# glacierbliss/iceberg_tracking_code

Hardware: AMD Instinct MI355X
Metric: frame_pairs_per_sec (higher is better)
Workload: dtype u8/int32/f32

## Files before the change

### iceberg_tracking_code_amd/csrc/k_corners.hip

```cpp
#include <algorithm>
#include <cstdlib>

#include "icelk_internal.h"

namespace icelk {

namespace {

__device__ __forceinline__ int reflect101(int p, int n)
{
    if (n == 1) return 0;
    while (p < 0 || p >= n) p = p < 0 ? -p : 2 * n - 2 - p;
    return p;
}

__device__ __forceinline__ unsigned ordered_key(float v)
{
    const unsigned b = __float_as_uint(v);
    return (b & 0x80000000u) ? ~b : (b | 0x80000000u);
}
__device__ __forceinline__ float key_to_float(unsigned k)
{
    const unsigned b = (k & 0x80000000u) ? (k & 0x7fffffffu) : ~k;
    return __uint_as_float(b);
}

__device__ __forceinline__ unsigned pack_xy(int x, int y) { return ((unsigned)y << 16) | (unsigned)x; }

__device__ __forceinline__ float threshold_of(const unsigned* max_key, double quality)
{
    const unsigned mk = *max_key;
    const double max_val = mk ? (double)key_to_float(mk) : 0.0;
    return (float)(max_val * quality);
}

__device__ __forceinline__ float row_smooth(float a, float b, float c, float k0, float k1, int variant)
{
    if (variant & 2) return fmaf(k1, c, fmaf(k0, b, __fmul_rn(k1, a)));
    return __fadd_rn(__fadd_rn(__fmul_rn(k1, a), __fmul_rn(k0, b)), __fmul_rn(k1, c));
}

__device__ __forceinline__ void sobel_cov(float a0, float b0, float c0, float a1, float c1, float a2, float b2,
                                          float c2, float k0, float k1, float& xx, float& xy, float& yy, int variant = 0)
{
    const float dx = (variant & 1) ? fmaf(__fadd_rn(__fsub_rn(c0, a0), __fsub_rn(c2, a2)), k1, __fmul_rn(__fsub_rn(c1, a1), k0))
                                   : __fadd_rn(__fmul_rn(__fadd_rn(__fsub_rn(c0, a0), __fsub_rn(c2, a2)), k1),
                                               __fmul_rn(__fsub_rn(c1, a1), k0));
    const float t0 = row_smooth(a0, b0, c0, k0, k1, variant);
    const float t2 = row_smooth(a2, b2, c2, k0, k1, variant);
    const float dy = __fsub_rn(t2, t0);
    xx = __fmul_rn(dx, dx);
    xy = __fmul_rn(dx, dy);
    yy = __fmul_rn(dy, dy);
}

typedef float f2 __attribute__((ext_vector_type(2)));
__device__ __forceinline__ void sobel_cov2(f2 a0, f2 b0, f2 c0, f2 a1, f2 c1, f2 a2, f2 b2, f2 c2, float k0, float k1,
                                           f2& xx, f2& xy, f2& yy)
{
    const f2 dx = ((c0 - a0) + (c2 - a2)) * k1 + (c1 - a1) * k0;
    const f2 t0 = (a0 * k1 + b0 * k0) + c0 * k1;
    const f2 t2 = (a2 * k1 + b2 * k0) + c2 * k1;
    const f2 dy = t2 - t0;
    xx = dx * dx;
    xy = dx * dy;
    yy = dy * dy;
}

template <int N, int BS>
__device__ __forceinline__ void window_sums(const double (&v)[N + BS - 1], double (&out)[N])
{
    if constexpr (BS <= 3) {
#pragma unroll
        for (int i = 0; i < N; i++) {
            double s = 0;
#pragma unroll
            for (int k = 0; k < BS; k++) s += v[i + k];
            out[i] = s;
        }
    } else {
        double s = v[0];
#pragma unroll
        for (int k = 1; k < BS; k++) s += v[k];
        out[0] = s;
#pragma unroll
        for (int i = 1; i < N; i++) {
            s = (s - v[i - 1]) + v[i + BS - 1];
            out[i] = s;
        }
    }
}

__device__ __forceinline__ float min_eig_of(double s0, double s1, double s2, int variant = 0)
{
    const float a = __fmul_rn((float)s0, 0.5f), b = (float)s1, c = __fmul_rn((float)s2, 0.5f);
    const float d = __fsub_rn(a, c);
    const float r = (variant & 4) ? fmaf(b, b, __fmul_rn(d, d)) : __fadd_rn(__fmul_rn(d, d), __fmul_rn(b, b));
    return __fsub_rn(__fadd_rn(a, c), sqrtf(r));
}

__device__ __forceinline__ void publish_max(unsigned* max_key, unsigned best, int tid)
{
#pragma unroll
    for (int o = 32; o >= 1; o >>= 1) {
        const unsigned other = __shfl_xor(best, o);
        best = other > best ? other : best;
    }
    if ((tid & 63) == 0 && best > __atomic_load_n(max_key, __ATOMIC_RELAXED)) atomicMax(max_key, best);
}

struct CandSrc {
    const unsigned long long* keys;
    const int* blk_count;
    int nblk;
    int region;
};

constexpr int gcd_c(int a, int b) { return b == 0 ? a : gcd_c(b, a % b); }

template <int BS>
struct StripCfg {
    static constexpr int NT = 256;
    static constexpr int AN = BS / 2;
    static constexpr int EW = NT - (BS - 1);
    static constexpr int TW = EW - 2;
    static constexpr int R = 4;
    static constexpr int UNROLL = BS * R / gcd_c(BS, R);
    static constexpr int EH = (64 / UNROLL) * UNROLL;
    static constexpr int SH = EH - 2;
    static constexpr int NROWS = EH + BS - 1;
    static constexpr int RX = 4;
    static constexpr int NG = (EW + RX - 1) / RX;
    static constexpr int VP = NT + 2;
    static constexpr int SUB = 16, NSUB = (SH + SUB - 1) / SUB;
    static constexpr int V_BYTES = R * 3 * VP * 8;
    static constexpr int E_BYTES = 8 * NT * 4;
    static constexpr int LDS_BYTES = V_BYTES + E_BYTES;
    static_assert(EH % R == 0 && NG <= 64 && RX * NG <= NT + RX - 1, "one wave per row of a batch");
    static_assert(RX * (NG - 1) + RX + BS - 2 < VP, "row tasks stay inside a row of column sums");
    static_assert((VP * 8) % 16 == 0, "16-byte reads of the column sums");
};

struct SobelRoll {
    float d1, d2, t1, t2;
};

__device__ __forceinline__ float smooth3(float a, float b, float c, float k0, float k1)
{
    return __fadd_rn(__fadd_rn(__fmul_rn(k1, a), __fmul_rn(k0, b)), __fmul_rn(k1, c));
}

template <int BS, bool FRESH>
__device__ __forceinline__ void strip_body(const uint8_t* __restrict__ img, int w, int h, int pitch, float k0, float k1,
                                           const uint8_t* __restrict__ mask, int mask_pitch, unsigned* __restrict__ max_key,
                                           unsigned long long* __restrict__ raw, int* __restrict__ blk_count,
                                           float* __restrict__ eig_out, uint8_t* smem, int* s_cnt)
{
    using C = StripCfg<BS>;
    double* Vb = reinterpret_cast<double*>(smem);
    float* Er = reinterpret_cast<float*>(smem + C::V_BYTES);
    const int tid = threadIdx.x;
    const int x0 = blockIdx.x * C::TW, y0 = blockIdx.y * C::SH;
    const int xs = x0 - 1 - C::AN, ys = y0 - 1 - C::AN;
    const int rx = reflect101(xs + tid, w);
    const int xm = reflect101(rx - 1, w), xp = reflect101(rx + 1, w);
    const int bid = blockIdx.y * gridDim.x + blockIdx.x;
    if (tid < C::NSUB) s_cnt[tid] = 0;

    float ring[3][BS];
#pragma unroll
    for (int k = 0; k < BS; k++) ring[0][k] = ring[1][k] = ring[2][k] = 0.f;
    double V[3] = {0.0, 0.0, 0.0};
    SobelRoll S{};
    unsigned pa = 0, pb = 0, pc = 0;
    if (!FRESH) {
        const uint8_t* r2 = img + (size_t)(ys - 1) * pitch;
        const uint8_t* r1 = r2 + pitch;
        const uint8_t* r0 = r1 + pitch;
        const float a2 = (float)r2[xm], b2 = (float)r2[rx], c2 = (float)r2[xp];
        const float a1 = (float)r1[xm], b1 = (float)r1[rx], c1 = (float)r1[xp];
        S.d2 = __fsub_rn(c2, a2); S.t2 = smooth3(a2, b2, c2, k0, k1);
        S.d1 = __fsub_rn(c1, a1); S.t1 = smooth3(a1, b1, c1, k0, k1);
        pa = r0[xm]; pb = r0[rx]; pc = r0[xp];
    }
    auto cov_row = [&](int r, float& xx, float& xy, float& yy) {
        float dtop, dmid, dbot, ttop, tbot;
        if (FRESH) {
            const int ry = reflect101(ys + r, h);
            const uint8_t* q0 = img + (size_t)reflect101(ry - 1, h) * pitch;
            const uint8_t* q1 = img + (size_t)ry * pitch;
            const uint8_t* q2 = img + (size_t)reflect101(ry + 1, h) * pitch;
            const float a0 = (float)q0[xm], b0 = (float)q0[rx], c0 = (float)q0[xp];
            const float a1 = (float)q1[xm], c1 = (float)q1[xp];
            const float a2 = (float)q2[xm], b2 = (float)q2[rx], c2 = (float)q2[xp];
            dtop = __fsub_rn(c0, a0); dmid = __fsub_rn(c1, a1); dbot = __fsub_rn(c2, a2);
            ttop = smooth3(a0, b0, c0, k0, k1); tbot = smooth3(a2, b2, c2, k0, k1);
        } else {
            const float a = (float)pa, b = (float)pb, c = (float)pc;
            int nr = ys + r + 2;
            nr = nr < h ? nr : h - 1;
            const uint8_t* q = img + (size_t)nr * pitch;
            pa = q[xm]; pb = q[rx]; pc = q[xp];
            dtop = S.d2; dmid = S.d1; dbot = __fsub_rn(c, a);
            ttop = S.t2; tbot = smooth3(a, b, c, k0, k1);
            S.d2 = S.d1; S.d1 = dbot; S.t2 = S.t1; S.t1 = tbot;
        }
        const float dx = __fadd_rn(__fmul_rn(__fadd_rn(dtop, dbot), k1), __fmul_rn(dmid, k0));
        const float dy = __fsub_rn(tbot, ttop);
        xx = __fmul_rn(dx, dx); xy = __fmul_rn(dx, dy); yy = __fmul_rn(dy, dy);
    };

#pragma unroll
    for (int r = 0; r < BS - 1; r++) {
        float p[3];
        cov_row(r, p[0], p[1], p[2]);
#pragma unroll
        for (int q = 0; q < 3; q++) { V[q] += (double)p[q]; ring[q][r] = p[q]; }
    }

    unsigned best = 0;
    const int wr = tid >> 6, g = tid & 63;
    for (int base = 0; base < C::EH; base += C::UNROLL) {
#pragma unroll
        for (int j = 0; j < C::UNROLL; j++) {
            const int i = base + j;
            const int K = (BS - 1 + j) % BS;
            float p[3];
            cov_row(BS - 1 + i, p[0], p[1], p[2]);
#pragma unroll
            for (int q = 0; q < 3; q++) {
                V[q] = (V[q] + (double)p[q]) - (double)ring[q][K];
                ring[q][K] = p[q];
                Vb[((j % C::R) * 3 + q) * C::VP + tid] = V[q];
            }
            __builtin_amdgcn_sched_barrier(0);
            if (j % C::R != C::R - 1) continue;
            const int eb = i / C::R;
            __syncthreads();
            if (g < C::NG && wr < C::R) {
                double Sm[3][C::RX];
#pragma unroll
                for (int q = 0; q < 3; q++) {
                    double v[C::RX + BS - 1];
                    const double* src = Vb + (wr * 3 + q) * C::VP + C::RX * g;
#pragma unroll
                    for (int k = 0; k < C::RX + BS - 1; k++) v[k] = src[k];
                    window_sums<C::RX, BS>(v, Sm[q]);
                    __builtin_amdgcn_sched_barrier(0);
                }
                const int er = eb * C::R + wr;
                float e[C::RX];
#pragma unroll
                for (int k = 0; k < C::RX; k++) e[k] = min_eig_of(Sm[0][k], Sm[1][k], Sm[2][k]);
                *reinterpret_cast<float4*>(Er + (er & 7) * C::NT + C::RX * g) = make_float4(e[0], e[1], e[2], e[3]);
                const int y = y0 - 1 + er;
                if (er >= 1 && er <= C::SH && y < h) {
#pragma unroll
                    for (int k = 0; k < C::RX; k++) {
                        const int ce = C::RX * g + k, x = x0 - 1 + ce;
                        if (ce >= 1 && ce <= C::TW && x < w) {
                            if (eig_out) eig_out[(size_t)y * w + x] = e[k];
                            if (!mask || mask[(size_t)y * mask_pitch + x]) {
                                const unsigned key = ordered_key(e[k]);
                                best = key > best ? key : best;
                            }
                        }
                    }
                }
            }
            __syncthreads();
            {
                const int x = x0 - 1 + tid;
                if (tid >= 1 && tid <= C::TW && x >= 1 && x < w - 1) {
                    float m3[6], mid[6], side[6];
#pragma unroll
                    for (int k = 0; k < 6; k++) {
                        const float* row = Er + ((eb * C::R - 2 + k) & 7) * C::NT + tid;
                        const float l = row[-1], c = row[0], r = row[1];
                        mid[k] = c;
                        side[k] = fmaxf(l, r);
                        m3[k] = fmaxf(side[k], c);
                    }
#pragma unroll
                    for (int q = 0; q < 4; q++) {
                        const int c = eb * C::R - 1 + q, y = y0 - 1 + c;
                        if (c < 1 || c > C::SH || y < 1 || y >= h - 1) continue;
                        const float v = mid[q + 1];
                        if (!(v > 0.f)) continue;
                        const float m = fmaxf(fmaxf(m3[q], m3[q + 2]), side[q + 1]);
                        if (v < m) continue;
                        if (mask && !mask[(size_t)y * mask_pitch + x]) continue;
                        const int sub = (c - 1) / C::SUB;
                        const int pos = atomicAdd(&s_cnt[sub], 1);
                        raw[((size_t)bid * C::NSUB + sub) * (C::TW * C::SUB) + pos] =
                            ((unsigned long long)ordered_key(v) << 32) | pack_xy(x, y);
                    }
                }
            }
        }
    }
    publish_max(max_key, best, tid);
    __syncthreads();
    if (tid < C::NSUB) blk_count[bid * C::NSUB + tid] = s_cnt[tid];
}

template <int BS>
__global__ __launch_bounds__(256) __attribute__((amdgpu_waves_per_eu(3, 4))) void k_eig_strip(const uint8_t* __restrict__ img, int w, int h, int pitch, float k0,
                                                    float k1, const uint8_t* __restrict__ mask, int mask_pitch,
                                                    unsigned* __restrict__ max_key,
                                                    unsigned long long* __restrict__ raw, int* __restrict__ blk_count,
                                                    float* __restrict__ eig_out)
{
    using C = StripCfg<BS>;
    extern __shared__ __attribute__((aligned(16))) uint8_t smem[];
    __shared__ int s_cnt[C::NSUB];
    const int ys = (int)blockIdx.y * C::SH - 1 - C::AN;
    if (ys - 1 >= 0 && ys + C::NROWS <= h - 1)
        strip_body<BS, false>(img, w, h, pitch, k0, k1, mask, mask_pitch, max_key, raw, blk_count, eig_out, smem, s_cnt);
    else
        strip_body<BS, true>(img, w, h, pitch, k0, k1, mask, mask_pitch, max_key, raw, blk_count, eig_out, smem, s_cnt);
}

__device__ __forceinline__ void block_append(bool keep, unsigned long long key, unsigned long long* out,
                                             int* out_count, int* s_cnt, int* s_base)
{
    if (threadIdx.x == 0) *s_cnt = 0;
    __syncthreads();
    const int pos = keep ? atomicAdd(s_cnt, 1) : 0;
    __syncthreads();
    if (threadIdx.x == 0 && *s_cnt) *s_base = atomicAdd(out_count, *s_cnt);
    __syncthreads();
    if (keep) out[*s_base + pos] = key;
    __syncthreads();
}

__global__ __launch_bounds__(256) void k_flatten(CandSrc src, const unsigned* __restrict__ max_key, double quality,
                                                 unsigned long long* __restrict__ cand, int* __restrict__ cand_count)
{
    __shared__ int s_cnt, s_base;
    const float thr = threshold_of(max_key, quality);
    for (int b = blockIdx.x; b < src.nblk; b += gridDim.x) {
        const int cnt = src.blk_count[b];
        for (int i0 = 0; i0 < cnt; i0 += 256) {
            const int i = i0 + threadIdx.x;
            unsigned long long key = 0;
            bool keep = false;
            if (i < cnt) {
                key = src.keys[(size_t)b * src.region + i];
                keep = key_to_float((unsigned)(key >> 32)) > thr;
            }
            block_append(keep, key, cand, cand_count, &s_cnt, &s_base);
        }
    }
}

constexpr int EIG_TW = 64;
constexpr int EIG_TH = 16;

__global__ __launch_bounds__(256) void k_min_eig(const uint8_t* __restrict__ img, int w, int h, int pitch, int bs,
                                                 float k0, float k1, float* __restrict__ eig,
                                                 const uint8_t* __restrict__ mask, int mask_pitch,
                                                 unsigned* __restrict__ max_key, int variant)
{
    extern __shared__ __attribute__((aligned(16))) uint8_t smem[];
    const int anchor = bs / 2;
    const int ew = EIG_TW + bs - 1, eh = EIG_TH + bs - 1;
    double* hs = reinterpret_cast<double*>(smem);
    float* cov = reinterpret_cast<float*>(smem + sizeof(double) * 3 * eh * EIG_TW);
    const int x0 = blockIdx.x * EIG_TW, y0 = blockIdx.y * EIG_TH;
    const int tid = threadIdx.x;
    for (int i = tid; i < ew * eh; i += 256) {
        const int ey = i / ew, ex = i - ey * ew;
        const int rx = reflect101(x0 - anchor + ex, w), ry = reflect101(y0 - anchor + ey, h);
        const int xm = reflect101(rx - 1, w), xp = reflect101(rx + 1, w);
        const int ym = reflect101(ry - 1, h), yp = reflect101(ry + 1, h);
        const uint8_t* r0 = img + (size_t)ym * pitch;
        const uint8_t* r1 = img + (size_t)ry * pitch;
        const uint8_t* r2 = img + (size_t)yp * pitch;
        float xx, xy, yy;
        sobel_cov((float)r0[xm], (float)r0[rx], (float)r0[xp], (float)r1[xm], (float)r1[xp], (float)r2[xm],
                  (float)r2[rx], (float)r2[xp], k0, k1, xx, xy, yy, variant);
        cov[i] = xx;
        cov[ew * eh + i] = xy;
        cov[2 * ew * eh + i] = yy;
    }
    __syncthreads();
    for (int i = tid; i < eh * EIG_TW; i += 256) {
        const int ey = i / EIG_TW, ox = i - ey * EIG_TW;
        const float* c = cov + ey * ew + ox;
        double s0 = 0, s1 = 0, s2 = 0;
        for (int k = 0; k < bs; k++) {
            s0 += (double)c[k];
            s1 += (double)c[ew * eh + k];
            s2 += (double)c[2 * ew * eh + k];
        }
        hs[i] = s0;
        hs[eh * EIG_TW + i] = s1;
        hs[2 * eh * EIG_TW + i] = s2;
    }
    __syncthreads();
    unsigned best = 0;
    for (int i = tid; i < EIG_TH * EIG_TW; i += 256) {
        const int oy = i / EIG_TW, ox = i - oy * EIG_TW;
        const int x = x0 + ox, y = y0 + oy;
        if (x >= w || y >= h) continue;
        const double* r = hs + oy * EIG_TW + ox;
        double s0 = 0, s1 = 0, s2 = 0;
        for (int k = 0; k < bs; k++) {
            s0 += r[k * EIG_TW];
            s1 += r[eh * EIG_TW + k * EIG_TW];
            s2 += r[2 * eh * EIG_TW + k * EIG_TW];
        }
        const float v = min_eig_of(s0, s1, s2, variant);
        eig[(size_t)y * w + x] = v;
        if (!mask || mask[(size_t)y * mask_pitch + x]) {
            const unsigned k = ordered_key(v);
            best = k > best ? k : best;
        }
    }
    publish_max(max_key, best, tid);
}

constexpr int NMS_ROWS = 8;
__global__ __launch_bounds__(256) void k_nms_collect(const float* __restrict__ eig, int w, int h,
                                                     const uint8_t* __restrict__ mask, int mask_pitch,
                                                     const unsigned* __restrict__ max_key, double quality,
                                                     unsigned long long* __restrict__ raw, int* __restrict__ blk_count)
{
    __shared__ int list_n;
    const int tid = threadIdx.x;
    if (tid == 0) list_n = 0;
    __syncthreads();
    const int bid = blockIdx.y * gridDim.x + blockIdx.x;
    unsigned long long* region = raw + (size_t)bid * (256 * NMS_ROWS);
    const float thr = threshold_of(max_key, quality);
    const int x = blockIdx.x * 256 + tid + 1;
    for (int r = 0; r < NMS_ROWS; r++) {
        const int y = blockIdx.y * NMS_ROWS + r + 1;
        if (x >= w - 1 || y >= h - 1) continue;
        const float v = eig[(size_t)y * w + x];
        if (!(v > thr) || v == 0.f) continue;
        if (mask && !mask[(size_t)y * mask_pitch + x]) continue;
        float m = 0.f;
#pragma unroll
        for (int dy = -1; dy <= 1; dy++)
#pragma unroll
            for (int dx = -1; dx <= 1; dx++) {
                float q = eig[(size_t)(y + dy) * w + (x + dx)];
                q = q > thr ? q : 0.f;
                m = q > m ? q : m;
            }
        if (v != m) continue;
        region[atomicAdd(&list_n, 1)] = ((unsigned long long)ordered_key(v) << 32) | pack_xy(x, y);
    }
    __syncthreads();
    if (tid == 0) blk_count[bid] = list_n;
}

constexpr int CT = 64;
constexpr int SCAN_CHUNK = 2048;
constexpr int CHUNK_TOT_STRIDE = 32;

__device__ __forceinline__ void chunk_add(int* __restrict__ chunk_tot, bool active, int chunk)
{
    unsigned long long pending = __ballot(active);
    while (pending) {
        const int leader = __ffsll((long long)pending) - 1;
        const int c = __shfl(chunk, leader);
        const unsigned long long same = __ballot(active && chunk == c) & pending;
        if ((int)threadIdx.x == leader) atomicAdd(&chunk_tot[c * CHUNK_TOT_STRIDE], __popcll(same));
        pending &= ~same;
    }
}

__global__ __launch_bounds__(CT) void k_cell_count(CandSrc src, const unsigned* __restrict__ max_key, double quality,
                                                   const unsigned* __restrict__ prune_key, int w, int cell, int gw,
                                                   int* __restrict__ cell_count, int* __restrict__ chunk_tot)
{
    const float thr = threshold_of(max_key, quality);
    const unsigned pk = *prune_key;
    for (int b = blockIdx.x; b < src.nblk; b += gridDim.x) {
        const int cnt = src.blk_count[b];
        for (int i0 = 0; i0 < cnt; i0 += CT) {
            const int i = i0 + threadIdx.x;
            bool keep = false;
            int c = 0;
            if (i < cnt) {
                const unsigned long long key = src.keys[(size_t)b * src.region + i];
                keep = (unsigned)(key >> 32) >= pk && key_to_float((unsigned)(key >> 32)) > thr;
                const unsigned idx = (unsigned)key;
                const int y = (int)(idx >> 16), x = (int)(idx & 0xffffu);
                c = (y / cell) * gw + (x / cell);
            }
            if (keep) atomicAdd(&cell_count[c], 1);
            chunk_add(chunk_tot, keep, c / SCAN_CHUNK);
        }
    }
}

constexpr int KEY_SHIFT = 18;
constexpr int KEY_BINS = 2048;
__device__ __forceinline__ int key_bin(unsigned key, unsigned max_key)
{
    const int b = (int)(max_key >> KEY_SHIFT) - (int)(key >> KEY_SHIFT);
    return b < 0 ? 0 : (b >= KEY_BINS ? KEY_BINS - 1 : b);
}

__global__ __launch_bounds__(CT) void k_key_hist(CandSrc src, const unsigned* __restrict__ max_key, double quality,
                                                 unsigned* __restrict__ hist)
{
    __shared__ unsigned lh[KEY_BINS];
    for (int i = threadIdx.x; i < KEY_BINS; i += CT) lh[i] = 0;
    __syncthreads();
    const float thr = threshold_of(max_key, quality);
    const unsigned mk = *max_key;
    for (int b = blockIdx.x; b < src.nblk; b += gridDim.x) {
        const int cnt = src.blk_count[b];
        for (int i = threadIdx.x; i < cnt; i += CT) {
            const unsigned k = (unsigned)(src.keys[(size_t)b * src.region + i] >> 32);
            if (key_to_float(k) > thr) atomicAdd(&lh[key_bin(k, mk)], 1u);
        }
    }
    __syncthreads();
    for (int i = threadIdx.x; i < KEY_BINS; i += CT) {
        const unsigned v = lh[i];
        if (v) atomicAdd(&hist[i], v);
    }
}

__global__ __launch_bounds__(CT) void k_key_select(const unsigned* __restrict__ hist, unsigned want,
                                                   const unsigned* __restrict__ max_key,
                                                   unsigned* __restrict__ prune_key)
{
    constexpr int PER = KEY_BINS / CT;
    const int lane = threadIdx.x;
    unsigned s = 0;
    for (int i = 0; i < PER; i++) s += hist[lane * PER + i];
    unsigned incl = s;
#pragma unroll
    for (int o = 1; o < CT; o <<= 1) {
        const unsigned v = __shfl_up(incl, o);
        if (lane >= o) incl += v;
    }
    const unsigned total = __shfl(incl, CT - 1);
    if (lane == 0 && total < want) *prune_key = 0u;
    const unsigned above = incl - s;
    if (above < want && incl >= want) {
        unsigned run = above;
        for (int i = 0; i < PER; i++) {
            run += hist[lane * PER + i];
            if (run >= want) {
                const int bin = lane * PER + i;
                const int top = (int)(*max_key >> KEY_SHIFT);
                *prune_key = (bin >= KEY_BINS - 1 || top - bin <= 0) ? 0u : (unsigned)(top - bin) << KEY_SHIFT;
                break;
            }
        }
    }
}

__global__ __launch_bounds__(CT) void k_scan(const int* __restrict__ count, const int* __restrict__ chunk_tot,
                                             int* __restrict__ start, int n)
{
    const int lane = threadIdx.x;
    const int lo = blockIdx.x * SCAN_CHUNK;
    int run = 0;
    for (int c = lane; c < (int)blockIdx.x; c += CT) run += chunk_tot[c * CHUNK_TOT_STRIDE];
#pragma unroll
    for (int o = 32; o >= 1; o >>= 1) run += __shfl_xor(run, o);
    for (int r = 0; r < SCAN_CHUNK / (4 * CT); r++) {
        const int i0 = lo + r * 4 * CT + 4 * lane;
        int c[4], s = 0;
#pragma unroll
        for (int k = 0; k < 4; k++) {
            c[k] = i0 + k < n ? count[i0 + k] : 0;
            s += c[k];
        }
        int inc = s;
#pragma unroll
        for (int o = 1; o < CT; o <<= 1) {
            const int v = __shfl_up(inc, o);
            if (lane >= o) inc += v;
        }
        int at = run + inc - s;
#pragma unroll
        for (int k = 0; k < 4; k++) {
            if (i0 + k < n) start[i0 + k] = at;
            at += c[k];
            if (i0 + k == n - 1) start[n] = at;
        }
        run += __shfl(inc, CT - 1);
    }
    if (n == 0 && blockIdx.x == 0 && lane == 0) start[0] = 0;
}

__global__ __launch_bounds__(CT) void k_cell_fill(CandSrc src, const unsigned* __restrict__ max_key, double quality,
                                                   const unsigned* __restrict__ prune_key, int w, int cell, int gw,
                                                   const int* __restrict__ cell_start, int* __restrict__ cell_fill,
                                                   unsigned long long* __restrict__ cell_cand,
                                                   uint8_t* __restrict__ state)
{
    const float thr = threshold_of(max_key, quality);
    const unsigned pk = *prune_key;
    for (int b = blockIdx.x; b < src.nblk; b += gridDim.x) {
        const int cnt = src.blk_count[b];
        for (int i = threadIdx.x; i < cnt; i += CT) {
            const unsigned long long key = src.keys[(size_t)b * src.region + i];
            if ((unsigned)(key >> 32) < pk || !(key_to_float((unsigned)(key >> 32)) > thr)) continue;
            const unsigned idx = (unsigned)key;
            const int y = (int)(idx >> 16), x = (int)(idx & 0xffffu);
            const int c = (y / cell) * gw + (x / cell);
            const int pos = cell_start[c] + atomicAdd(&cell_fill[c], 1);
            cell_cand[pos] = key;
            state[pos] = 0;
        }
    }
}

constexpr int SUP_K = 24;
constexpr int SUP_SPINS = 48;
__global__ __launch_bounds__(CT) void k_suppress(const unsigned long long* __restrict__ cell_cand,
                                                  const int* __restrict__ n_ptr, int cell, int gw, int gh,
                                                  const int* __restrict__ cell_start, uint8_t* state, double md2,
                                                  int* __restrict__ launch_counters, int r)
{
    __shared__ int blockers[SUP_K * CT];
    if (r > 0 && launch_counters[r - 1] == 0) return;
    const int n = *n_ptr;
    int* mine = blockers + threadIdx.x;
    for (int i = blockIdx.x * blockDim.x + threadIdx.x; i < n; i += gridDim.x * blockDim.x) {
        if (__atomic_load_n(&state[i], __ATOMIC_RELAXED)) continue;
        const unsigned long long key = cell_cand[i];
        const unsigned idx = (unsigned)key;
        const int y = (int)(idx >> 16), x = (int)(idx & 0xffffu);
        const int xc = x / cell, yc = y / cell;
        const int x1 = max(0, xc - 1), y1 = max(0, yc - 1), x2 = min(gw - 1, xc + 1), y2 = min(gh - 1, yc + 1);
        int cnt = 0;
        bool rejected = false, overflow = false;
        for (int yy = y1; yy <= y2 && !rejected; yy++) {
            const int b = cell_start[yy * gw + x1], e = cell_start[yy * gw + x2 + 1];
            for (int j = b; j < e; j++) {
                const unsigned long long kj = cell_cand[j];
                if (kj <= key) continue;
                const unsigned ij = (unsigned)kj;
                const int yj = (int)(ij >> 16), xj = (int)(ij & 0xffffu);
                const float dx = (float)(x - xj), dy = (float)(y - yj);
                if (!((double)(dx * dx + dy * dy) < md2)) continue;
                const uint8_t sj = __atomic_load_n(&state[j], __ATOMIC_RELAXED);
                if (sj == 1) { rejected = true; break; }
                if (sj == 0) {
                    if (cnt < SUP_K) mine[CT * cnt++] = j;
                    else overflow = true;
                }
            }
        }
        bool decided = false;
        if (rejected) { __atomic_store_n(&state[i], (uint8_t)2, __ATOMIC_RELAXED); decided = true; }
        else if (cnt == 0 && !overflow) { __atomic_store_n(&state[i], (uint8_t)1, __ATOMIC_RELAXED); decided = true; }
        for (int spin = 0; spin < SUP_SPINS && !decided && !overflow; spin++) {
            __builtin_amdgcn_s_sleep(8);
            int k = 0;
            for (int q = 0; q < cnt; q++) {
                const int j = mine[CT * q];
                const uint8_t sj = __atomic_load_n(&state[j], __ATOMIC_RELAXED);
                if (sj == 1) { rejected = true; break; }
                if (sj == 0) mine[CT * k++] = j;
            }
            cnt = k;
            if (rejected) { __atomic_store_n(&state[i], (uint8_t)2, __ATOMIC_RELAXED); decided = true; }
            else if (cnt == 0) { __atomic_store_n(&state[i], (uint8_t)1, __ATOMIC_RELAXED); decided = true; }
        }
        if (!decided) atomicAdd(&launch_counters[r], 1);
    }
}

__global__ void k_detect_reset(int* __restrict__ cell_count, int* __restrict__ cell_fill, int ncell,
                               int* __restrict__ chunk_tot, int* __restrict__ undecided, int* __restrict__ acc_count,
                               int* __restrict__ cand_count, unsigned* __restrict__ max_key,
                               unsigned* __restrict__ key_hist, unsigned* __restrict__ prune_key, int full)
{
    const int i0 = blockIdx.x * blockDim.x + threadIdx.x;
    for (int i = i0; i <= ncell; i += gridDim.x * blockDim.x) {
        cell_count[i] = 0;
        if (i < ncell) cell_fill[i] = 0;
        if (i % SCAN_CHUNK == 0) chunk_tot[(i / SCAN_CHUNK) * CHUNK_TOT_STRIDE] = 0;
    }
    if (full & 1)
        for (int i = i0; i < KEY_BINS; i += gridDim.x * blockDim.x) key_hist[i] = 0;
    if (i0 < 8) undecided[i0] = 0;
    if (i0 == 0) {
        *acc_count = 0;
        *cand_count = 0;
        *prune_key = 0;
        if (full & 2) *max_key = 0;
    }
}

__global__ __launch_bounds__(CT) void k_gather_accepted(const unsigned long long* __restrict__ cell_cand,
                                                         const int* __restrict__ n_ptr,
                                                         const uint8_t* __restrict__ state,
                                                         unsigned long long* __restrict__ acc,
                                                         int* __restrict__ acc_count)
{
    __shared__ int s_cnt, s_base;
    const int n = *n_ptr;
    for (int i0 = blockIdx.x * CT; i0 < n; i0 += gridDim.x * CT) {
        const int i = i0 + threadIdx.x;
        const bool keep = i < n && state[i] == 1;
        block_append(keep, keep ? cell_cand[i] : 0ull, acc, acc_count, &s_cnt, &s_base);
    }
}

__global__ void k_emit(const unsigned long long* __restrict__ keys, int n, int w, float* __restrict__ xy)
{
    const int i = blockIdx.x * blockDim.x + threadIdx.x;
    if (i >= n) return;
    const unsigned idx = (unsigned)keys[i];
    const int y = (int)(idx >> 16), x = (int)(idx & 0xffffu);
    xy[2 * i] = (float)x;
    xy[2 * i + 1] = (float)y;
}

__global__ __launch_bounds__(CT) void k_tail(const unsigned long long* __restrict__ keys, int n, float* __restrict__ corners,
                                             float* __restrict__ seg_xy, uint8_t* __restrict__ seg_alive,
                                             float* __restrict__ seg_tracks, int max_vert, int emit_blocks,
                                             int* __restrict__ cell_count, int* __restrict__ cell_fill, int ncell,
                                             int* __restrict__ chunk_tot, int* __restrict__ undecided,
                                             int* __restrict__ acc_count, int* __restrict__ cand_count,
                                             unsigned* __restrict__ max_key, unsigned* __restrict__ key_hist,
                                             unsigned* __restrict__ prune_key, int full)
{
    if ((int)blockIdx.x < emit_blocks) {
        const int i = blockIdx.x * CT + threadIdx.x;
        if (i >= n) return;
        const unsigned idx = (unsigned)keys[i];
        const float x = (float)(int)(idx & 0xffffu), y = (float)(int)(idx >> 16);
        corners[2 * i] = x; corners[2 * i + 1] = y;
        seg_xy[2 * i] = x; seg_xy[2 * i + 1] = y;
        seg_alive[i] = 1;
        seg_tracks[((size_t)i * max_vert) * 2] = x;
        seg_tracks[((size_t)i * max_vert) * 2 + 1] = y;
        return;
    }
    const int i0 = ((int)blockIdx.x - emit_blocks) * CT + threadIdx.x, stride = ((int)gridDim.x - emit_blocks) * CT;
    for (int i = i0; i <= ncell; i += stride) {
        cell_count[i] = 0;
        if (i < ncell) cell_fill[i] = 0;
        if (i % SCAN_CHUNK == 0) chunk_tot[(i / SCAN_CHUNK) * CHUNK_TOT_STRIDE] = 0;
    }
    if (full & 1)
        for (int i = i0; i < KEY_BINS; i += stride) key_hist[i] = 0;
    if (i0 < 8) undecided[i0] = 0;
    if (i0 == 0) {
        *acc_count = 0;
        *cand_count = 0;
        *prune_key = 0;
        if (full & 2) *max_key = 0;
    }
}

void sobel_scale(int block_size, float* k0, float* k1)
{
    double scale = (double)(1 << 2) * block_size;
    scale *= 255.0;
    scale = 1.0 / scale;
    *k1 = (float)(1.0 * scale);
    *k0 = (float)(2.0 * scale);
}

template <int BS>
void launch_strip(hipStream_t s, const Level& img, float k0, float k1, const uint8_t* mask, int mask_pitch,
                  unsigned* max_key, unsigned long long* raw, int* blk_count, float* eig_out, CandSrc* src)
{
    using C = StripCfg<BS>;
    dim3 grid((img.w + C::TW - 1) / C::TW, (img.h + C::SH - 1) / C::SH);
    hipLaunchKernelGGL((k_eig_strip<BS>), grid, dim3(C::NT), C::LDS_BYTES, s, img.ptr, img.w, img.h, img.pitch, k0, k1, mask,
                       mask_pitch, max_key, raw, blk_count, eig_out);
    src->nblk = (int)(grid.x * grid.y) * C::NSUB;
    src->region = C::TW * C::SUB;
    src->keys = raw;
    src->blk_count = blk_count;
}

template <int BS>
void strip_geometry(int w, int h, size_t* regions, size_t* keys)
{
    using C = StripCfg<BS>;
    const size_t r = (size_t)((w + C::TW - 1) / C::TW) * ((h + C::SH - 1) / C::SH) * C::NSUB;
    const size_t k = r * (size_t)(C::TW * C::SUB);
    *regions = r > *regions ? r : *regions;
    *keys = k > *keys ? k : *keys;
}
void strip_layout(int w, int h, size_t* regions, size_t* keys)
{
    *regions = *keys = 0;
    strip_geometry<3>(w, h, regions, keys); strip_geometry<5>(w, h, regions, keys);
    strip_geometry<7>(w, h, regions, keys); strip_geometry<10>(w, h, regions, keys);
}

dim3 nms_grid(int w, int h) { return dim3((w - 2 + 255) / 256, (h - 2 + NMS_ROWS - 1) / NMS_ROWS); }

}

size_t min_eig_lds_bytes(int block_size)
{
    const int ew = EIG_TW + block_size - 1, eh = EIG_TH + block_size - 1;
    return sizeof(double) * 3 * eh * EIG_TW + sizeof(float) * 3 * eh * ew;
}

bool fused_block_size(int bs) { return bs == 3 || bs == 5 || bs == 7 || bs == 10; }

size_t candidate_capacity(int w, int h)
{
    size_t strip_r, strip_k;
    strip_layout(w, h, &strip_r, &strip_k);
    const size_t generic = (size_t)((w + 255) / 256) * ((h + NMS_ROWS - 1) / NMS_ROWS) * (256 * NMS_ROWS);
    const size_t m = std::max({generic, fast_key_capacity(w, h), strip_k});
    return m + 1024;
}
size_t candidate_blocks(int w, int h)
{
    size_t strip_r, strip_k;
    strip_layout(w, h, &strip_r, &strip_k);
    const dim3 g = nms_grid(w, h);
    const size_t m = std::max({(size_t)g.x * g.y, fast_regions(w, h), strip_r});
    return m + 16;
}

void launch_min_eig(hipStream_t s, const Level& img, int block_size, float* eig, const uint8_t* mask,
                    int mask_pitch, unsigned* max_key, int variant)
{
    float k0, k1;
    sobel_scale(block_size, &k0, &k1);
    const size_t lds = min_eig_lds_bytes(block_size);
    static size_t attr_lds = 0;
    if (lds > attr_lds) {
        hipFuncSetAttribute(reinterpret_cast<const void*>(&k_min_eig), hipFuncAttributeMaxDynamicSharedMemorySize,
                            (int)lds);
        attr_lds = lds;
    }
    dim3 grid((img.w + EIG_TW - 1) / EIG_TW, (img.h + EIG_TH - 1) / EIG_TH);
    hipLaunchKernelGGL(k_min_eig, grid, dim3(256), lds, s, img.ptr, img.w, img.h, img.pitch, block_size, k0, k1, eig,
                       mask, mask_pitch, max_key, variant);
}

static CandSrc src_of(const DetectScratch& D)
{
    CandSrc c;
    c.keys = D.raw;
    c.blk_count = D.blk_count;
    c.nblk = D.src_nblk;
    c.region = D.src_region;
    return c;
}

void launch_detect_reset(hipStream_t s, DetectScratch& D, int ncell, int mode)
{
    int blocks = (ncell + CT) / CT;
    if ((mode & 1) && blocks < KEY_BINS / CT) blocks = KEY_BINS / CT;
    if (blocks > 2048) blocks = 2048;
    hipLaunchKernelGGL(k_detect_reset, dim3(blocks), dim3(CT), 0, s, D.cell_count, D.cell_fill, ncell, D.chunk_tot, D.undecided,
                       D.acc_count, D.cand_count, D.max_key, D.key_hist, D.prune_key, mode);
}

void launch_candidates(hipStream_t s, DetectScratch& D, const Level& img, int block_size, const uint8_t* mask,
                       int mask_pitch, double quality, bool use_generic, float* eig_out_or_null, int variant)
{
    if (variant) use_generic = true;
    unsigned long long* raw = D.raw;
    CandSrc g_src{};
    const bool two_pass = D.acand != nullptr && getenv("ICELK_TWO_PASS_CORNERS") != nullptr;
    if (two_pass && !use_generic && fused_block_size(block_size) && !eig_out_or_null &&
        launch_candidates_fast(s, D, img, block_size, mask, mask_pitch, quality))
        return;
    if (!use_generic && fused_block_size(block_size)) {
        float k0, k1;
        sobel_scale(block_size, &k0, &k1);
        switch (block_size) {
            case 3: launch_strip<3>(s, img, k0, k1, mask, mask_pitch, D.max_key, raw, D.blk_count, eig_out_or_null, &g_src); break;
            case 5: launch_strip<5>(s, img, k0, k1, mask, mask_pitch, D.max_key, raw, D.blk_count, eig_out_or_null, &g_src); break;
            case 7: launch_strip<7>(s, img, k0, k1, mask, mask_pitch, D.max_key, raw, D.blk_count, eig_out_or_null, &g_src); break;
            default: launch_strip<10>(s, img, k0, k1, mask, mask_pitch, D.max_key, raw, D.blk_count, eig_out_or_null, &g_src); break;
        }
    } else {
        launch_min_eig(s, img, block_size, D.eig, mask, mask_pitch, D.max_key, variant);
        g_src.keys = raw;
        g_src.blk_count = D.blk_count;
        g_src.nblk = 0;
        g_src.region = 256 * NMS_ROWS;
        if (img.w >= 3 && img.h >= 3) {
            const dim3 grid = nms_grid(img.w, img.h);
            hipLaunchKernelGGL(k_nms_collect, grid, dim3(256), 0, s, D.eig, img.w, img.h, mask, mask_pitch, D.max_key,
                               quality, raw, D.blk_count);
            g_src.nblk = (int)(grid.x * grid.y);
        }
    }
    D.src_nblk = g_src.nblk;
    D.src_region = g_src.region;
}

void launch_flatten(hipStream_t s, DetectScratch& D, double quality)
{
    hipLaunchKernelGGL(k_flatten, dim3(512), dim3(256), 0, s, src_of(D), D.max_key, quality, D.cand, D.cand_count);
}

constexpr int kSuppressLaunches = 3;
static void suppress_launches(hipStream_t s, DetectScratch& D, int w, int h, double min_distance)
{
    const int cell = (int)lrint(min_distance);
    const int gw = (w + cell - 1) / cell, gh = (h + cell - 1) / cell;
    const double md2 = min_distance * min_distance;
    for (int r = 0; r < kSuppressLaunches; r++)
        hipLaunchKernelGGL(k_suppress, dim3(r < 2 ? 4096 : 512), dim3(CT), 0, s, D.cell_cand, D.cell_start + gw * gh, cell, gw, gh,
                           D.cell_start, D.state, md2, D.undecided, r);
}

static void gather_launch(hipStream_t s, DetectScratch& D, int ncell)
{
    hipLaunchKernelGGL(k_gather_accepted, dim3(1024), dim3(CT), 0, s, D.cell_cand, D.cell_start + ncell, D.state, D.acc,
                       D.acc_count);
}

TailReset tail_reset_of(DetectScratch& D, int ncell)
{
    TailReset r{};
    r.cell_count = D.cell_count;
    r.cell_fill = D.cell_fill;
    r.ncell = ncell;
    r.chunk_tot = D.chunk_tot;
    r.undecided = D.undecided;
    r.acc_count = D.acc_count;
    r.cand_count = D.cand_count;
    r.key_hist = D.key_hist;
    r.prune_key = D.prune_key;
    r.scan_chunk = SCAN_CHUNK;
    r.chunk_stride = CHUNK_TOT_STRIDE;
    r.key_bins = KEY_BINS;
    return r;
}

void launch_min_distance(hipStream_t s, DetectScratch& D, int w, int h, double min_distance, double quality,
                         int prune_want, bool no_gather)
{
    const int cell = (int)lrint(min_distance);
    const int gw = (w + cell - 1) / cell, gh = (h + cell - 1) / cell;
    const int ncell = gw * gh;
    if (prune_want > 0) {
        hipLaunchKernelGGL(k_key_hist, dim3(256), dim3(CT), 0, s, src_of(D), D.max_key, quality, D.key_hist);
        hipLaunchKernelGGL(k_key_select, dim3(1), dim3(CT), 0, s, D.key_hist, (unsigned)prune_want, D.max_key, D.prune_key);
    }
    hipLaunchKernelGGL(k_cell_count, dim3(4096), dim3(CT), 0, s, src_of(D), D.max_key, quality, D.prune_key, w, cell, gw,
                       D.cell_count, D.chunk_tot);
    hipLaunchKernelGGL(k_scan, dim3((ncell + SCAN_CHUNK - 1) / SCAN_CHUNK), dim3(CT), 0, s, D.cell_count, D.chunk_tot,
                       D.cell_start, ncell);
    hipLaunchKernelGGL(k_cell_fill, dim3(4096), dim3(CT), 0, s, src_of(D), D.max_key, quality, D.prune_key, w, cell, gw,
                       D.cell_start, D.cell_fill, D.cell_cand, D.state);
    suppress_launches(s, D, w, h, min_distance);
    if (!no_gather) gather_launch(s, D, ncell);
}

void continue_min_distance(hipStream_t s, DetectScratch& D, int w, int h, double min_distance)
{
    const int cell = (int)lrint(min_distance);
    const int ncell = ((w + cell - 1) / cell) * ((h + cell - 1) / cell);
    hipMemsetAsync(D.undecided, 0, sizeof(int) * 8, s);
    hipMemsetAsync(D.acc_count, 0, sizeof(int), s);
    suppress_launches(s, D, w, h, min_distance);
    gather_launch(s, D, ncell);
}

int suppress_launch_count() { return kSuppressLaunches; }

void launch_tail_fused(hipStream_t s, const unsigned long long* keys, int n, float* corners, float* seg_xy,
                       uint8_t* seg_alive, float* seg_tracks, int max_vert, DetectScratch& D, int ncell, int mode)
{
    const int emit_blocks = (n + CT - 1) / CT;
    int blocks = (ncell + CT) / CT;
    if ((mode & 1) && blocks < KEY_BINS / CT) blocks = KEY_BINS / CT;
    if (blocks > 2048) blocks = 2048;
    hipLaunchKernelGGL(k_tail, dim3(emit_blocks + blocks), dim3(CT), 0, s, keys, n, corners, seg_xy, seg_alive, seg_tracks,
                       max_vert, emit_blocks, D.cell_count, D.cell_fill, ncell, D.chunk_tot, D.undecided, D.acc_count,
                       D.cand_count, D.max_key, D.key_hist, D.prune_key, mode);
}

void launch_emit_corners(hipStream_t s, const unsigned long long* keys, int n, int w, float* xy)
{
    if (n <= 0) return;
    hipLaunchKernelGGL(k_emit, dim3((n + CT - 1) / CT), dim3(CT), 0, s, keys, n, w, xy);
}

}
```

Measured before the change: 7637.

## Micro-optimize Shi-Tomasi strip kernel with buffer loads, float max tracking, custom sqrt

Rewrites several inner-loop details of the fused corner strip kernel. Pixel reads now go through AMD buffer loads, with a fallback to the generic path when the image exceeds 4 GiB. The running maximum is tracked as a float using v_max and v_max3 instead of ordered integer keys. The hardware sqrt is paired with a correctly-rounded fixup, plane loads are reordered so LDS reads overlap the window sums, and occupancy hints change for smaller block sizes. Each change targets VALU and memory instruction count, at the cost of inline asm and a fixup path that must reproduce sqrtf rounding.

```diff
diff --git a/iceberg_tracking_code_amd/csrc/k_corners.hip b/iceberg_tracking_code_amd/csrc/k_corners.hip
--- a/iceberg_tracking_code_amd/csrc/k_corners.hip
+++ b/iceberg_tracking_code_amd/csrc/k_corners.hip
@@ -91,13 +91,61 @@
     }
 }
 
-__device__ __forceinline__ float min_eig_of(double s0, double s1, double s2, int variant = 0)
-{
-    const float a = __fmul_rn((float)s0, 0.5f), b = (float)s1, c = __fmul_rn((float)s2, 0.5f);
+__device__ __forceinline__ float sqrt_radicand(float x)
+{
+    const float xs = __fmul_rn(x, 0x1p64f);
+    const float s = __builtin_amdgcn_sqrtf(xs);
+    const float s_down = __int_as_float(__float_as_int(s) - 1), s_up = __int_as_float(__float_as_int(s) + 1);
+    const float r_down = __builtin_fmaf(-s_down, s, xs), r_up = __builtin_fmaf(-s_up, s, xs);
+    float r = r_down <= 0.f ? s_down : s;
+    r = r_up > 0.f ? s_up : r;
+    return __fmul_rn(r, 0x1p-32f);
+}
+
+__device__ __forceinline__ float min_eig_of(float s0, float s1, float s2, int variant = 0)
+{
+    const float a = __fmul_rn(s0, 0.5f), b = s1, c = __fmul_rn(s2, 0.5f);
     const float d = __fsub_rn(a, c);
     const float r = (variant & 4) ? fmaf(b, b, __fmul_rn(d, d)) : __fadd_rn(__fmul_rn(d, d), __fmul_rn(b, b));
-    return __fsub_rn(__fadd_rn(a, c), sqrtf(r));
-}
+    return __fsub_rn(__fadd_rn(a, c), sqrt_radicand(r));
+}
+
+__device__ __forceinline__ float vmax(float a, float b)
+{
+    float d;
+    asm("v_max_f32 %0, %1, %2" : "=v"(d) : "v"(a), "v"(b));
+    return d;
+}
+__device__ __forceinline__ float vmax3(float a, float b, float c)
+{
+    float d;
+    asm("v_max3_f32 %0, %1, %2, %3" : "=v"(d) : "v"(a), "v"(b), "v"(c));
+    return d;
+}
+
+__device__ __forceinline__ float byte_to_float(unsigned p)
+{
+    float f;
+    asm("v_cvt_f32_ubyte0 %0, %1" : "=v"(f) : "v"(p));
+    return f;
+}
+
+__device__ __forceinline__ unsigned key_of_running_max(float best)
+{
+    return best == -__builtin_inff() ? 0u : ordered_key(best);
+}
+
+struct PixelRows {
+    __amdgpu_buffer_rsrc_t rs;
+    unsigned pitch;
+    __device__ __forceinline__ PixelRows(const uint8_t* img, int pitch_, int h)
+        : rs(__builtin_amdgcn_make_buffer_rsrc(const_cast<uint8_t*>(img), 0, (int)((unsigned)pitch_ * (unsigned)h), 0x00020000)),
+          pitch((unsigned)pitch_) {}
+    __device__ __forceinline__ unsigned operator()(int row, int x) const
+    {
+        return __builtin_amdgcn_raw_buffer_load_b8(rs, x, (int)((unsigned)row * pitch), 0);
+    }
+};
 
 __device__ __forceinline__ void publish_max(unsigned* max_key, unsigned best, int tid)
 {
@@ -165,6 +213,7 @@
     const int rx = reflect101(xs + tid, w);
     const int xm = reflect101(rx - 1, w), xp = reflect101(rx + 1, w);
     const int bid = blockIdx.y * gridDim.x + blockIdx.x;
+    const PixelRows px(img, pitch, h);
     if (tid < C::NSUB) s_cnt[tid] = 0;
 
     float ring[3][BS];
@@ -174,33 +223,27 @@
     SobelRoll S{};
     unsigned pa = 0, pb = 0, pc = 0;
     if (!FRESH) {
-        const uint8_t* r2 = img + (size_t)(ys - 1) * pitch;
-        const uint8_t* r1 = r2 + pitch;
-        const uint8_t* r0 = r1 + pitch;
-        const float a2 = (float)r2[xm], b2 = (float)r2[rx], c2 = (float)r2[xp];
-        const float a1 = (float)r1[xm], b1 = (float)r1[rx], c1 = (float)r1[xp];
+        const float a2 = (float)px(ys - 1, xm), b2 = (float)px(ys - 1, rx), c2 = (float)px(ys - 1, xp);
+        const float a1 = (float)px(ys, xm), b1 = (float)px(ys, rx), c1 = (float)px(ys, xp);
         S.d2 = __fsub_rn(c2, a2); S.t2 = smooth3(a2, b2, c2, k0, k1);
         S.d1 = __fsub_rn(c1, a1); S.t1 = smooth3(a1, b1, c1, k0, k1);
-        pa = r0[xm]; pb = r0[rx]; pc = r0[xp];
+        pa = px(ys + 1, xm); pb = px(ys + 1, rx); pc = px(ys + 1, xp);
     }
     auto cov_row = [&](int r, float& xx, float& xy, float& yy) {
         float dtop, dmid, dbot, ttop, tbot;
         if (FRESH) {
             const int ry = reflect101(ys + r, h);
-            const uint8_t* q0 = img + (size_t)reflect101(ry - 1, h) * pitch;
-            const uint8_t* q1 = img + (size_t)ry * pitch;
-            const uint8_t* q2 = img + (size_t)reflect101(ry + 1, h) * pitch;
-            const float a0 = (float)q0[xm], b0 = (float)q0[rx], c0 = (float)q0[xp];
-            const float a1 = (float)q1[xm], c1 = (float)q1[xp];
-            const float a2 = (float)q2[xm], b2 = (float)q2[rx], c2 = (float)q2[xp];
+            const int q0 = reflect101(ry - 1, h), q2 = reflect101(ry + 1, h);
+            const float a0 = (float)px(q0, xm), b0 = (float)px(q0, rx), c0 = (float)px(q0, xp);
+            const float a1 = (float)px(ry, xm), c1 = (float)px(ry, xp);
+            const float a2 = (float)px(q2, xm), b2 = (float)px(q2, rx), c2 = (float)px(q2, xp);
             dtop = __fsub_rn(c0, a0); dmid = __fsub_rn(c1, a1); dbot = __fsub_rn(c2, a2);
             ttop = smooth3(a0, b0, c0, k0, k1); tbot = smooth3(a2, b2, c2, k0, k1);
         } else {
-            const float a = (float)pa, b = (float)pb, c = (float)pc;
+            const float a = byte_to_float(pa), b = byte_to_float(pb), c = byte_to_float(pc);
             int nr = ys + r + 2;
             nr = nr < h ? nr : h - 1;
-            const uint8_t* q = img + (size_t)nr * pitch;
-            pa = q[xm]; pb = q[rx]; pc = q[xp];
+            pa = px(nr, xm); pb = px(nr, rx); pc = px(nr, xp);
             dtop = S.d2; dmid = S.d1; dbot = __fsub_rn(c, a);
             ttop = S.t2; tbot = smooth3(a, b, c, k0, k1);
             S.d2 = S.d1; S.d1 = dbot; S.t2 = S.t1; S.t1 = tbot;
@@ -218,8 +261,8 @@
         for (int q = 0; q < 3; q++) { V[q] += (double)p[q]; ring[q][r] = p[q]; }
     }
 
-    unsigned best = 0;
-    const int wr = tid >> 6, g = tid & 63;
+    float best = -__builtin_inff();
+    const int wr = __builtin_amdgcn_readfirstlane(tid >> 6), g = tid & 63;
     for (int base = 0; base < C::EH; base += C::UNROLL) {
 #pragma unroll
         for (int j = 0; j < C::UNROLL; j++) {
@@ -238,15 +281,26 @@
             const int eb = i / C::R;
             __syncthreads();
             if (g < C::NG && wr < C::R) {
-                double Sm[3][C::RX];
+                float Sm[3][C::RX];
+                double v[3][C::RX + BS - 1];
+                auto load_plane = [&](int q) {
+                    const double* src = Vb + (wr * 3 + q) * C::VP + C::RX * g;
+#pragma unroll
+                    for (int k = 0; k < C::RX + BS - 1; k++) v[q][k] = src[k];
+                };
+                load_plane(0);
+                load_plane(1);
 #pragma unroll
                 for (int q = 0; q < 3; q++) {
-                    double v[C::RX + BS - 1];
-                    const double* src = Vb + (wr * 3 + q) * C::VP + C::RX * g;
-#pragma unroll
-                    for (int k = 0; k < C::RX + BS - 1; k++) v[k] = src[k];
-                    window_sums<C::RX, BS>(v, Sm[q]);
-                    __builtin_amdgcn_sched_barrier(0);
+                    double sums[C::RX];
+                    window_sums<C::RX, BS>(v[q], sums);
+#pragma unroll
+                    for (int k = 0; k < C::RX; k++) Sm[q][k] = (float)sums[k];
+                    if (q == 0) {
+#pragma unroll
+                        for (int k = 0; k < C::RX; k++) asm volatile("" : : "v"(Sm[q][k]) : "memory");
+                        load_plane(2);
+                    }
                 }
                 const int er = eb * C::R + wr;
                 float e[C::RX];
@@ -260,10 +314,7 @@
                         const int ce = C::RX * g + k, x = x0 - 1 + ce;
                         if (ce >= 1 && ce <= C::TW && x < w) {
                             if (eig_out) eig_out[(size_t)y * w + x] = e[k];
-                            if (!mask || mask[(size_t)y * mask_pitch + x]) {
-                                const unsigned key = ordered_key(e[k]);
-                                best = key > best ? key : best;
-                            }
+                            if (!mask || mask[(size_t)y * mask_pitch + x]) best = vmax(best, e[k]);
                         }
                     }
                 }
@@ -278,8 +329,8 @@
                         const float* row = Er + ((eb * C::R - 2 + k) & 7) * C::NT + tid;
                         const float l = row[-1], c = row[0], r = row[1];
                         mid[k] = c;
-                        side[k] = fmaxf(l, r);
-                        m3[k] = fmaxf(side[k], c);
+                        side[k] = vmax(l, r);
+                        m3[k] = vmax3(l, r, c);
                     }
 #pragma unroll
                     for (int q = 0; q < 4; q++) {
@@ -287,7 +338,7 @@
                         if (c < 1 || c > C::SH || y < 1 || y >= h - 1) continue;
                         const float v = mid[q + 1];
                         if (!(v > 0.f)) continue;
-                        const float m = fmaxf(fmaxf(m3[q], m3[q + 2]), side[q + 1]);
+                        const float m = vmax3(m3[q], m3[q + 2], side[q + 1]);
                         if (v < m) continue;
                         if (mask && !mask[(size_t)y * mask_pitch + x]) continue;
                         const int sub = (c - 1) / C::SUB;
@@ -299,13 +350,13 @@
             }
         }
     }
-    publish_max(max_key, best, tid);
+    publish_max(max_key, key_of_running_max(best), tid);
     __syncthreads();
     if (tid < C::NSUB) blk_count[bid * C::NSUB + tid] = s_cnt[tid];
 }
 
 template <int BS>
-__global__ __launch_bounds__(256) __attribute__((amdgpu_waves_per_eu(3, 4))) void k_eig_strip(const uint8_t* __restrict__ img, int w, int h, int pitch, float k0,
+__global__ __launch_bounds__(256) __attribute__((amdgpu_waves_per_eu(BS == 10 ? 3 : 4, 4))) void k_eig_strip(const uint8_t* __restrict__ img, int w, int h, int pitch, float k0,
                                                     float k1, const uint8_t* __restrict__ mask, int mask_pitch,
                                                     unsigned* __restrict__ max_key,
                                                     unsigned long long* __restrict__ raw, int* __restrict__ blk_count,
@@ -411,7 +462,7 @@
             s1 += r[eh * EIG_TW + k * EIG_TW];
             s2 += r[2 * eh * EIG_TW + k * EIG_TW];
         }
-        const float v = min_eig_of(s0, s1, s2, variant);
+        const float v = min_eig_of((float)s0, (float)s1, (float)s2, variant);
         eig[(size_t)y * w + x] = v;
         if (!mask || mask[(size_t)y * mask_pitch + x]) {
             const unsigned k = ordered_key(v);
@@ -867,6 +918,7 @@
                        int mask_pitch, double quality, bool use_generic, float* eig_out_or_null, int variant)
 {
     if (variant) use_generic = true;
+    if ((unsigned long long)img.pitch * (unsigned long long)img.h >= (1ull << 32)) use_generic = true;
     unsigned long long* raw = D.raw;
     CandSrc g_src{};
     const bool two_pass = D.acand != nullptr && getenv("ICELK_TWO_PASS_CORNERS") != nullptr;
```

After: 7381. -3.4%, worse.
